# Alexandre-nk-Perdereau/video-fingerprint

Measured on NVIDIA B200. Metric: fingerprint videos/s (64 frames@64^2), higher is better.
Workload: dtype bf16

## Files before the change

### video_fingerprint_b200/csrc/stem_common.cuh

```cuda
#pragma once
#include "conv1_kernel.cuh"
#include "epilogues.cuh"

namespace vfp {

constexpr int kStemThreads = 768;
constexpr int kStemEpiWarp0 = 4, kStemEpiWarps = 8;
constexpr int kStemABuf = 9 * 16 * 128;
constexpr int kStemUnitBytes = 2 * kStemABuf;
constexpr int kStemWBlocks = 5;
constexpr int kStemRawSlotBytes = 8192;
constexpr int kStemTilePitch = 72;
constexpr int kStemTileBytes = 29184;
static_assert((67 * kStemTilePitch + 8) * 6 <= kStemTileBytes, "HWC tile");

template <int N> __device__ __forceinline__ void setmaxnreg_inc() { asm volatile("setmaxnreg.inc.sync.aligned.u32 %0;" ::"n"(N)); }
template <int N> __device__ __forceinline__ void setmaxnreg_dec() { asm volatile("setmaxnreg.dec.sync.aligned.u32 %0;" ::"n"(N)); }

__device__ __forceinline__ uint32_t relu_pack_bf16x2(float lo, float hi) {
  uint32_t d;
  asm("cvt.rn.relu.bf16x2.f32 %0, %1, %2;" : "=r"(d) : "f"(hi), "f"(lo));
  return d;
}
__device__ __forceinline__ void bulk_copy_g2s(void* dst, const void* src, uint32_t bytes, uint64_t* bar) {
  asm volatile("cp.async.bulk.shared::cluster.global.mbarrier::complete_tx::bytes [%0], [%1], %2, [%3];" ::"r"(smem_u32(dst)),
               "l"(reinterpret_cast<uint64_t>(src)), "r"(bytes), "r"(smem_u32(bar))
               : "memory");
}
__device__ __forceinline__ void bulk_prefetch_l2(const void* src, uint32_t bytes) {
  asm volatile("cp.async.bulk.prefetch.L2.global [%0], %1;" ::"l"(reinterpret_cast<uint64_t>(src)), "r"(bytes) : "memory");
}
__device__ __forceinline__ uint32_t u8x2_to_bf16x2(uint32_t lo, uint32_t hi) {
  return pack_bf16x2((float)lo * (1.0f / 255.0f), (float)hi * (1.0f / 255.0f));
}

__device__ __forceinline__ void stem_transpose_frame(const uint8_t* const (&pl)[3], uint8_t* tile, int frame_dtype, int ltid,
                                                     int n_threads) {
  if (frame_dtype == kFrameBF16) {
    for (int i = ltid; i < 512; i += n_threads) {
      const int h = i >> 3, w0 = (i & 7) * 8;
      const uint4 a = *reinterpret_cast<const uint4*>(pl[0] + (h * 64 + w0) * 2);
      const uint4 b = *reinterpret_cast<const uint4*>(pl[1] + (h * 64 + w0) * 2);
      const uint4 c = *reinterpret_cast<const uint4*>(pl[2] + (h * 64 + w0) * 2);
      uint4* dst = reinterpret_cast<uint4*>(tile + (h + 2) * (kStemTilePitch * 6) + (w0 + 8) * 6);
      uint4 o0, o1, o2;
      o0.x = __byte_perm(a.x, b.x, 0x5410); o0.y = __byte_perm(c.x, a.x, 0x7610); o0.z = __byte_perm(b.x, c.x, 0x7632);
      o0.w = __byte_perm(a.y, b.y, 0x5410); o1.x = __byte_perm(c.y, a.y, 0x7610); o1.y = __byte_perm(b.y, c.y, 0x7632);
      o1.z = __byte_perm(a.z, b.z, 0x5410); o1.w = __byte_perm(c.z, a.z, 0x7610); o2.x = __byte_perm(b.z, c.z, 0x7632);
      o2.y = __byte_perm(a.w, b.w, 0x5410); o2.z = __byte_perm(c.w, a.w, 0x7610); o2.w = __byte_perm(b.w, c.w, 0x7632);
      dst[0] = o0; dst[1] = o1; dst[2] = o2;
    }
  } else if (frame_dtype == kFrameU8) {
    for (int i = ltid; i < 512; i += n_threads) {
      const int h = i >> 3, w0 = (i & 7) * 8;
      const uint2 a = *reinterpret_cast<const uint2*>(pl[0] + h * 64 + w0);
      const uint2 b = *reinterpret_cast<const uint2*>(pl[1] + h * 64 + w0);
      const uint2 c = *reinterpret_cast<const uint2*>(pl[2] + h * 64 + w0);
      uint4* dst = reinterpret_cast<uint4*>(tile + (h + 2) * (kStemTilePitch * 6) + (w0 + 8) * 6);
      uint32_t o[12];
#pragma unroll
      for (int half = 0; half < 2; ++half) {
        const uint32_t av = half ? a.y : a.x, bv = half ? b.y : b.x, cv = half ? c.y : c.x;
#pragma unroll
        for (int pp = 0; pp < 2; ++pp) {
          const uint32_t a0 = (av >> (16 * pp)) & 0xFF, a1 = (av >> (16 * pp + 8)) & 0xFF;
          const uint32_t b0 = (bv >> (16 * pp)) & 0xFF, b1 = (bv >> (16 * pp + 8)) & 0xFF;
          const uint32_t c0 = (cv >> (16 * pp)) & 0xFF, c1 = (cv >> (16 * pp + 8)) & 0xFF;
          o[half * 6 + pp * 3 + 0] = u8x2_to_bf16x2(a0, b0);
          o[half * 6 + pp * 3 + 1] = u8x2_to_bf16x2(c0, a1);
          o[half * 6 + pp * 3 + 2] = u8x2_to_bf16x2(b1, c1);
        }
      }
      dst[0] = make_uint4(o[0], o[1], o[2], o[3]);
      dst[1] = make_uint4(o[4], o[5], o[6], o[7]);
      dst[2] = make_uint4(o[8], o[9], o[10], o[11]);
    }
  } else {
    for (int i = ltid; i < 768; i += n_threads) {
      const int byte0 = i * 16;
      const int chunk = byte0 >> 12;
      const uint4 q = *reinterpret_cast<const uint4*>((chunk == 0 ? pl[0] : chunk == 1 ? pl[1] : pl[2]) + (byte0 & 4095));
      const int h = byte0 / 192, off = byte0 - h * 192;
      uint4* dst = reinterpret_cast<uint4*>(tile + (h + 2) * (kStemTilePitch * 6) + 48 + 2 * off);
      const uint32_t w[4] = {q.x, q.y, q.z, q.w};
      uint32_t o[8];
#pragma unroll
      for (int j = 0; j < 4; ++j) {
        o[2 * j] = u8x2_to_bf16x2(w[j] & 0xFF, (w[j] >> 8) & 0xFF);
        o[2 * j + 1] = u8x2_to_bf16x2((w[j] >> 16) & 0xFF, w[j] >> 24);
      }
      dst[0] = make_uint4(o[0], o[1], o[2], o[3]);
      dst[1] = make_uint4(o[4], o[5], o[6], o[7]);
    }
  }
}

}
```

### video_fingerprint_b200/csrc/stem_ts_kernel.cuh

```cuda
#pragma once
#include "stem_common.cuh"

namespace vfp {

constexpr int kTsGenWarp0 = 12, kTsGenWarps = 4;
constexpr int kTsEpiWarp0 = 16, kTsEpiWarps = 4;
constexpr int kTsRawSlots = 3;
constexpr int kTsXposeWarp1 = 20, kTsXposeWarps = 5;
constexpr int kTsABufs = 2;
constexpr int kTsColAcc = 0, kTsColA = 256, kTsColD = 384;
#ifndef VFP_STEM_HALFB
#define VFP_STEM_HALFB 0
#endif
#ifndef VFP_STEM_KNOCKOUT
#define VFP_STEM_KNOCKOUT 0
#endif
constexpr int kTsKnock = VFP_STEM_KNOCKOUT;

struct StemTsSmem {
  static constexpr int kC1 = 0;
  static constexpr int kW2 = kC1 + 2 * kStemUnitBytes;
  static constexpr int kW1 = kW2 + kStemWBlocks * 8192;
  static constexpr int kStage = kW1 + 2 * 8192;
  static constexpr int kRaw = kStage + kStemEpiWarps * 2048;
  static constexpr int kTile = kRaw + kTsRawSlots * kStemRawSlotBytes;
  static constexpr int kBars = kTile + 2 * kStemTileBytes;
  static constexpr int kBias = kBars + 512;
  static constexpr int kTotal = kBias + 256 + 1024;
};
static_assert(StemTsSmem::kTotal <= 232448, "stem TS kernel shared memory");
static_assert(StemTsSmem::kW2 % 1024 == 0 && StemTsSmem::kW1 % 1024 == 0 && StemTsSmem::kStage % 1024 == 0 && StemTsSmem::kRaw % 1024 == 0,
              "alignment");

struct StemTsParams {
  alignas(64) CUtensorMap tmap_w2;
  alignas(64) CUtensorMap tmap_w1;
  alignas(64) CUtensorMap tmap_out;
  const unsigned long long* frame_addr;
  int frame_dtype;
  long long n_frames;
  const float* c2_bias;
};

constexpr uint32_t kDescHiSw128 = (uint32_t)(((8ull * 128) >> 4) | (1ull << 14) | (2ull << 29));
__device__ __forceinline__ uint32_t desc_lo_sw128(uint32_t smem_addr) { return ((smem_addr & 0x3FFFFu) >> 4) | (1u << 16); }

template <bool ACC>
__device__ __forceinline__ void umma_ss_lo(uint32_t tmem_d, uint32_t adesc_lo, uint32_t bdesc_lo, uint32_t idesc) {
  asm volatile(
      "{\n\t"
      ".reg .pred p;\n\t"
      ".reg .b64 da, db;\n\t"
      "setp.ne.b32 p, %5, 0;\n\t"
      "mov.b64 da, {%1, %4};\n\t"
      "mov.b64 db, {%2, %4};\n\t"
      "tcgen05.mma.cta_group::1.kind::f16 [%0], da, db, %3, p;\n\t"
      "}\n" ::"r"(tmem_d),
      "r"(adesc_lo), "r"(bdesc_lo), "r"(idesc), "r"(kDescHiSw128), "r"(ACC ? 1u : 0u)
      : "memory");
}
template <bool ACC>
__device__ __forceinline__ void umma_ts_lo(uint32_t tmem_d, uint32_t tmem_a, uint32_t bdesc_lo, uint32_t idesc) {
  asm volatile(
      "{\n\t"
      ".reg .pred p;\n\t"
      ".reg .b64 db;\n\t"
      "setp.ne.b32 p, %5, 0;\n\t"
      "mov.b64 db, {%2, %4};\n\t"
      "tcgen05.mma.cta_group::1.kind::f16 [%0], [%1], db, %3, p;\n\t"
      "}\n" ::"r"(tmem_d),
      "r"(tmem_a), "r"(bdesc_lo), "r"(idesc), "r"(kDescHiSw128), "r"(ACC ? 1u : 0u)
      : "memory");
}
__device__ __forceinline__ void tmem_st_32x32(uint32_t taddr, const uint32_t* v) {
  asm volatile(
      "tcgen05.st.sync.aligned.32x32b.x32.b32 [%0], "
      "{%1, %2, %3, %4, %5, %6, %7, %8, %9, %10, %11, %12, %13, %14, %15, %16, "
      "%17, %18, %19, %20, %21, %22, %23, %24, %25, %26, %27, %28, %29, %30, %31, %32};" ::"r"(taddr),
      "r"(v[0]), "r"(v[1]), "r"(v[2]), "r"(v[3]), "r"(v[4]), "r"(v[5]), "r"(v[6]), "r"(v[7]), "r"(v[8]), "r"(v[9]), "r"(v[10]),
      "r"(v[11]), "r"(v[12]), "r"(v[13]), "r"(v[14]), "r"(v[15]), "r"(v[16]), "r"(v[17]), "r"(v[18]), "r"(v[19]), "r"(v[20]),
      "r"(v[21]), "r"(v[22]), "r"(v[23]), "r"(v[24]), "r"(v[25]), "r"(v[26]), "r"(v[27]), "r"(v[28]), "r"(v[29]), "r"(v[30]),
      "r"(v[31])
      : "memory");
}
__device__ __forceinline__ void tmem_st_wait() { asm volatile("tcgen05.wait::st.sync.aligned;" ::: "memory"); }

__global__ void __launch_bounds__(kStemThreads, 1) stem_ts_kernel(const __grid_constant__ StemTsParams p) {
  extern __shared__ uint8_t smem_raw[];
  uint8_t* smem = smem_raw + ((1024u - (smem_u32(smem_raw) & 1023u)) & 1023u);
  uint8_t* c1buf = smem + StemTsSmem::kC1;
  uint8_t* w2buf = smem + StemTsSmem::kW2;
  uint8_t* w1buf = smem + StemTsSmem::kW1;
  uint8_t* stagebuf = smem + StemTsSmem::kStage;
  uint8_t* rawbuf = smem + StemTsSmem::kRaw;
  uint8_t* tilebuf = smem + StemTsSmem::kTile;
  uint64_t* bars = reinterpret_cast<uint64_t*>(smem + StemTsSmem::kBars);
  uint64_t* w_full = bars;
  uint64_t* c1_full = bars + 1;
  uint64_t* c1_empty = bars + 3;
  uint64_t* acc_full = bars + 28;
  uint64_t* acc_empty = bars + 30;
  uint64_t* tile_full = bars + 7;
  uint64_t* tile_empty = bars + 9;
  uint64_t* a_full = bars + 11;
  uint64_t* a_empty = bars + 14;
  uint64_t* d_full = bars + 17;
  uint64_t* d_empty = bars + 19;
  uint64_t* raw_full = bars + 32;
  uint64_t* raw_empty = bars + 37;
  uint32_t* tmem_slot = reinterpret_cast<uint32_t*>(bars + 42);
  float* c2_bias_s = reinterpret_cast<float*>(smem + StemTsSmem::kBias);

  const int tid = threadIdx.x;
  const int warp = tid >> 5, lane = tid & 31;
  pdl_launch_dependents();
  const int n_local = (p.n_frames > blockIdx.x) ? (int)((p.n_frames - blockIdx.x + gridDim.x - 1) / gridDim.x) : 0;
  const int n_tiles = 4 * n_local, n_units = 2 * n_local;

  for (int i = tid; i < (2 * kStemUnitBytes) / 16; i += kStemThreads) reinterpret_cast<uint4*>(c1buf)[i] = make_uint4(0, 0, 0, 0);
  for (int i = tid; i < (2 * kStemTileBytes) / 16; i += kStemThreads) reinterpret_cast<uint4*>(tilebuf)[i] = make_uint4(0, 0, 0, 0);
  if (tid < 64) c2_bias_s[tid] = __ldg(p.c2_bias + tid);
  if (warp == 0 && lane == 0) {
    tma_prefetch_desc(&p.tmap_w2);
    tma_prefetch_desc(&p.tmap_w1);
    tma_prefetch_desc(&p.tmap_out);
    mbar_init(w_full, 1);
    mbar_init(&c1_full[0], 2 * kTsEpiWarps);
    mbar_init(&c1_full[1], 2 * kTsEpiWarps + 1);
    for (int i = 0; i < 2; ++i) {
      mbar_init(&c1_empty[i], 1);
      mbar_init(&acc_full[i], 1);
      mbar_init(&acc_empty[i], kStemEpiWarps);
      mbar_init(&tile_full[i], kTsXposeWarps);
      mbar_init(&tile_empty[i], kTsGenWarps);
      mbar_init(&d_full[i], 1);
      mbar_init(&d_empty[i], kTsEpiWarps);
    }
    for (int i = 0; i < kTsABufs; ++i) {
      mbar_init(&a_full[i], kTsGenWarps);
      mbar_init(&a_empty[i], 1);
    }
    for (int i = 0; i < kTsRawSlots; ++i) {
      mbar_init(&raw_full[i], 1);
      mbar_init(&raw_empty[i], kTsXposeWarps);
    }
    fence_mbar_init();
  }
  if (warp == 1) {
    tmem_alloc(tmem_slot, 512);
    tmem_relinquish();
  }
  fence_proxy_async_smem();
  tc_fence_before();
  __syncthreads();
  tc_fence_after();
  const uint32_t tmem_base = *tmem_slot;
  const uint32_t plane_bytes = p.frame_dtype == kFrameBF16 ? 8192u : 4096u;
  pdl_wait();

  auto transposer_role = [&](int ltid) {
    int slot0 = 0;
    uint32_t n0 = 0;
    for (int li = 0; li < n_local; ++li) {
      const int t = li & 1;
      uint8_t* tile = tilebuf + t * kStemTileBytes;
      mbar_wait_lazy(&tile_empty[t], (uint32_t)(((li >> 1) & 1) ^ 1));
      const uint8_t* pl[3];
#pragma unroll
      for (int c = 0; c < 3; ++c) {
        const uint32_t n = n0 + c;
        const int s = (slot0 + c) % kTsRawSlots;
        mbar_wait_lazy(&raw_full[s], (n / kTsRawSlots) & 1u);
        pl[c] = rawbuf + s * kStemRawSlotBytes;
      }
      if (!(kTsKnock & 2)) stem_transpose_frame(pl, tile, p.frame_dtype, ltid, kTsXposeWarps * 32);
      __syncwarp();
      if (lane == 0) {
#pragma unroll
        for (int c = 0; c < 3; ++c) mbar_arrive(&raw_empty[(slot0 + c) % kTsRawSlots]);
        mbar_arrive(&tile_full[t]);
      }
      slot0 = (slot0 + 3) % kTsRawSlots;
      n0 += 3;
    }
  };

  if (warp < kStemEpiWarp0) {
    setmaxnreg_dec<56>();
    if (warp == 0) {
      if (lane == 0) {
        mbar_arrive_expect_tx(w_full, (kStemWBlocks + 2) * 8192);
        for (int kb = 0; kb < kStemWBlocks; ++kb) tma_load_2d(&p.tmap_w2, w_full, w2buf + kb * 8192, kb * 64, 0);
        for (int kb = 0; kb < 2; ++kb) tma_load_2d(&p.tmap_w1, w_full, w1buf + kb * 8192, kb * 64, 0);
        const unsigned long long* addr = p.frame_addr + blockIdx.x;
        int slot = 0;
        uint32_t ph = 0;
        for (int li = 0; li < n_local; ++li) {
          const uint8_t* src = reinterpret_cast<const uint8_t*>(__ldg(addr + (size_t)li * gridDim.x));
          if (li + 2 < n_local && !(kTsKnock & 4))
            bulk_prefetch_l2(reinterpret_cast<const uint8_t*>(__ldg(addr + (size_t)(li + 2) * gridDim.x)), 3 * plane_bytes);
          for (int c = 0; c < 3; ++c) {
            mbar_wait_lazy(&raw_empty[slot], ph ^ 1);
            if (kTsKnock & 4) {
              mbar_arrive(&raw_full[slot]);
            } else {
              mbar_arrive_expect_tx(&raw_full[slot], plane_bytes);
              bulk_copy_g2s(rawbuf + slot * kStemRawSlotBytes, src + c * plane_bytes, plane_bytes, &raw_full[slot]);
            }
            if (++slot == kTsRawSlots) { slot = 0; ph ^= 1; }
          }
        }
      }
    } else if (warp == 1) {
      constexpr uint32_t idesc64 = umma_idesc_bf16(128, VFP_STEM_HALFB ? 32 : 64);
      mbar_wait_relaxed(w_full, 0);
      const uint32_t w1_lo = desc_lo_sw128(smem_u32(w1buf));
      int ab = 0;
      uint32_t aph = 0;
      for (int g = 0; g < n_tiles; ++g) {
        const int b = g & 1;
        const uint32_t ph = (uint32_t)((g >> 1) & 1);
        mbar_wait_relaxed(&a_full[ab], aph);
        mbar_wait_relaxed(&d_empty[b], ph ^ 1);
        tc_fence_after();
        if (lane == 0) {
          const uint32_t a_col = tmem_base + kTsColA + ab * 64, d_col = tmem_base + kTsColD + b * 64;
          if (!(kTsKnock & 16)) {
            umma_ts_lo<false>(d_col, a_col, w1_lo, idesc64);
#pragma unroll
            for (int s = 1; s < 8; ++s) umma_ts_lo<true>(d_col, a_col + 8 * s, w1_lo + (s >> 2) * 512 + 2 * (s & 3), idesc64);
          }
          umma_commit(&a_empty[ab]);
          umma_commit(&d_full[b]);
        }
        __syncwarp();
        if (++ab == kTsABufs) { ab = 0; aph ^= 1; }
      }
    } else if (warp == 3) {
      constexpr uint32_t idesc64 = umma_idesc_bf16(128, VFP_STEM_HALFB ? 32 : 64);
      constexpr uint32_t idesc128 = umma_idesc_bf16(128, VFP_STEM_HALFB ? 64 : 128);
      mbar_wait_relaxed(w_full, 0);
      const uint32_t w2_lo = desc_lo_sw128(smem_u32(w2buf));
      const uint32_t c1_lo = desc_lo_sw128(smem_u32(c1buf));
      for (int u = 0; u < n_units; ++u) {
        const int b = u & 1;
        const uint32_t ph = (uint32_t)((u >> 1) & 1);
        mbar_wait_relaxed(&acc_empty[b], ph ^ 1);
        mbar_wait_relaxed(&c1_full[b], ph);
        tc_fence_after();
        if (lane == 0) {
          const uint32_t d_acc = tmem_base + kTsColAcc + b * 128;
          const uint32_t al0 = c1_lo + b * (kStemUnitBytes >> 4), al1 = al0 + (kStemABuf >> 4);
          if (!(kTsKnock & 8)) {
            umma_ss_lo<false>(d_acc, al1 + 128, w2_lo + 512, idesc128);
            umma_ss_lo<true>(d_acc, al0 + 128, w2_lo, idesc64);
#pragma unroll
            for (int k = 1; k < 4; ++k) {
              umma_ss_lo<true>(d_acc, al0 + 128 + 2 * k, w2_lo + 2 * k, idesc64);
              umma_ss_lo<true>(d_acc, al1 + 128 + 2 * k, w2_lo + 512 + 2 * k, idesc128);
            }
#pragma unroll
            for (int k = 0; k < 2; ++k) {
              umma_ss_lo<true>(d_acc, al0 + 2 * (2 + k), w2_lo + 3 * 512 + 2 * (2 + k), idesc64);
              umma_ss_lo<true>(d_acc, al1 + 2 * k, w2_lo + 3 * 512 + 2 * k, idesc128);
            }
          }
          umma_commit(&c1_empty[b]);
          umma_commit(&acc_full[b]);
        }
        __syncwarp();
      }
    } else {
      transposer_role(lane);
    }
  } else if (warp < kTsGenWarp0) {
    setmaxnreg_dec<56>();
    const int quarter = warp & 3;
    const int col_half = (warp - kStemEpiWarp0) >> 2;
    const float keep = (lane & 15) == 0 ? 0.0f : 1.0f;
    const float2 keep2 = make_float2(keep, keep);
    const uint32_t taddr = tmem_base + (static_cast<uint32_t>(quarter * 32) << 16) + kTsColAcc + col_half * 32;
    uint8_t* dst = stagebuf + (warp - kStemEpiWarp0) * 2048;
    uint8_t* r0 = dst + lane * 64;
    const int sw = (lane >> 1) & 3;
    int out_row = (int)blockIdx.x * 256 + quarter * 32;
    for (int u = 0; u < n_units; ++u) {
      const int b = u & 1;
      mbar_wait_relaxed(&acc_full[b], (uint32_t)((u >> 1) & 1));
      tc_fence_after();
      if (lane == 0) tma_store_wait_read<0>();
      __syncwarp();
      if (kTsKnock & 128) {
        tc_fence_before();
        __syncwarp();
        if (lane == 0) mbar_arrive(&acc_empty[b]);
        continue;
      }
      uint32_t va[2][8], vb[2][8];
      tmem_ld_32x8(taddr + b * 128, va[0]);
      tmem_ld_32x8(taddr + b * 128 + 64, vb[0]);
#pragma unroll
      for (int c = 0; c < 4; ++c) {
        uint32_t(&v0)[8] = va[c & 1];
        uint32_t(&v2)[8] = vb[c & 1];
        tmem_ld_wait();
        if (c < 3) {
          tmem_ld_32x8(taddr + b * 128 + 8 * (c + 1), va[(c + 1) & 1]);
          tmem_ld_32x8(taddr + b * 128 + 64 + 8 * (c + 1), vb[(c + 1) & 1]);
        } else {
          tc_fence_before();
          __syncwarp();
          if (lane == 0) mbar_arrive(&acc_empty[b]);
        }
        uint32_t q[4];
#pragma unroll
        for (int i = 0; i < 8; i += 4) {
          const float4 bb = *reinterpret_cast<const float4*>(c2_bias_s + col_half * 32 + 8 * c + i);
          const float s0 = __shfl_up_sync(0xffffffffu, __uint_as_float(v2[i]), 1), s1 = __shfl_up_sync(0xffffffffu, __uint_as_float(v2[i + 1]), 1);
          const float s2 = __shfl_up_sync(0xffffffffu, __uint_as_float(v2[i + 2]), 1), s3 = __shfl_up_sync(0xffffffffu, __uint_as_float(v2[i + 3]), 1);
          const float2 y01 = ffma2(make_float2(s0, s1), keep2, fadd2(make_float2(__uint_as_float(v0[i]), __uint_as_float(v0[i + 1])), make_float2(bb.x, bb.y)));
          const float2 y23 = ffma2(make_float2(s2, s3), keep2, fadd2(make_float2(__uint_as_float(v0[i + 2]), __uint_as_float(v0[i + 3])), make_float2(bb.z, bb.w)));
          q[i / 2] = relu_pack_bf16x2(y01.x, y01.y);
          q[i / 2 + 1] = relu_pack_bf16x2(y23.x, y23.y);
        }
        *reinterpret_cast<uint4*>(r0 + ((c ^ sw) << 4)) = make_uint4(q[0], q[1], q[2], q[3]);
      }
      fence_proxy_async_smem();
      __syncwarp();
      if (lane == 0 && !(kTsKnock & 1)) {
        tma_store_2d(&p.tmap_out, dst, col_half * 32, out_row + (u & 1) * 128);
        tma_store_commit();
      }
      if (u & 1) out_row += (int)gridDim.x * 256;
    }
    if (lane == 0) tma_store_wait_read<0>();
  } else if (warp < kTsEpiWarp0) {
    setmaxnreg_inc<112>();
    const int q = warp & 3;
    const int cx = lane & 15, sh = lane >> 4;
    const uint32_t lane_base = tmem_base + (static_cast<uint32_t>(q * 32) << 16) + kTsColA;
    const uint8_t* lane_src = tilebuf + ((4 * q + 2 * sh) * 108 + 6 * cx + 8) * 4;
    int ab = 0;
    uint32_t aph = 0;
    for (int li = 0; li < n_local; ++li) {
      mbar_wait_relaxed(&tile_full[li & 1], (uint32_t)((li >> 1) & 1));
#pragma unroll 1
      for (int t = 0; t < 4; ++t) {
        const uint2* src = reinterpret_cast<const uint2*>(lane_src + (li & 1) * kStemTileBytes + t * (16 * 108 * 4));
        uint32_t v[64];
#pragma unroll
        for (int kh = 0; kh < 5; ++kh)
#pragma unroll
          for (int j = 0; j < 6; ++j) {
            const uint2 w = (kTsKnock & 64) ? make_uint2(0u, 0u) : src[kh * 54 + j];
            v[kh * 12 + 2 * j] = w.x;
            v[kh * 12 + 2 * j + 1] = w.y;
          }
        v[60] = 0x3F803F80u;
        v[61] = 0u; v[62] = 0u; v[63] = 0u;
        if (t == 3) {
          __syncwarp();
          if (lane == 0) mbar_arrive(&tile_empty[li & 1]);
        }
        mbar_wait_relaxed(&a_empty[ab], aph ^ 1);
        tc_fence_after();
        if (!(kTsKnock & 512)) {
          tmem_st_32x32(lane_base + ab * 64, v);
          tmem_st_32x32(lane_base + ab * 64 + 32, v + 32);
          tmem_st_wait();
        }
        tc_fence_before();
        __syncwarp();
        if (lane == 0) mbar_arrive(&a_full[ab]);
        if (++ab == kTsABufs) { ab = 0; aph ^= 1; }
      }
    }
  } else if (warp < kTsEpiWarp0 + kTsEpiWarps) {
    setmaxnreg_inc<96>();
    const int q = warp & 3;
    const int cx = lane & 15, sh = lane >> 4;
    const uint32_t lane_base = tmem_base + (static_cast<uint32_t>(q * 32) << 16) + kTsColD;
    const uint32_t phase = (uint32_t)(cx & 7);
    uint32_t chunk_off[2][4];
#pragma unroll
    for (int sw = 0; sw < 2; ++sw)
#pragma unroll
      for (int j = 0; j < 4; ++j) chunk_off[sw][j] = (((uint32_t)((sh ^ sw) * 4 + j)) ^ phase) << 4;
    for (int g = 0; g < n_tiles; ++g) {
      const int li = g >> 2;
      const int b = g & 1;
      const int hf = (g >> 1) & 1;
      const int cyu = 4 * (g & 1) + q;
      mbar_wait_relaxed(&d_full[b], (uint32_t)((g >> 1) & 1));
      tc_fence_after();
      uint32_t packed[2][16];
#pragma unroll
      for (int sw = 0; sw < 2; ++sw) {
        if (kTsKnock & 256) break;
        uint32_t d[32];
        tmem_ld_32x32(lane_base + b * 64 + sw * 32, d);
        tmem_ld_wait();
#pragma unroll
        for (int j = 0; j < 16; ++j) packed[sw][j] = relu_pack_bf16x2(__uint_as_float(d[2 * j]), __uint_as_float(d[2 * j + 1]));
      }
      tc_fence_before();
      __syncwarp();
      if (lane == 0) mbar_arrive(&d_empty[b]);
      mbar_wait_relaxed(&c1_empty[hf], (uint32_t)((li & 1) ^ 1));
      uint8_t* row = c1buf + hf * kStemUnitBytes + ((cyu + 1) * 16 + cx) * 128;
      if (!(kTsKnock & 32)) {
#pragma unroll
        for (int sw = 0; sw < 2; ++sw)
#pragma unroll
          for (int j = 0; j < 4; ++j)
            *reinterpret_cast<uint4*>(row + sw * kStemABuf + chunk_off[sw][j]) =
                make_uint4(packed[sw][4 * j], packed[sw][4 * j + 1], packed[sw][4 * j + 2], packed[sw][4 * j + 3]);
      }
      const bool halo = hf == 0 && cyu == 7;
      if (halo) {
        mbar_wait_relaxed(&c1_empty[1], (uint32_t)((li & 1) ^ 1));
        uint8_t* hrow = c1buf + kStemUnitBytes + cx * 128;
#pragma unroll
        for (int sw = 0; sw < 2; ++sw)
#pragma unroll
          for (int j = 0; j < 4; ++j)
            *reinterpret_cast<uint4*>(hrow + sw * kStemABuf + chunk_off[sw][j]) =
                make_uint4(packed[sw][4 * j], packed[sw][4 * j + 1], packed[sw][4 * j + 2], packed[sw][4 * j + 3]);
      }
      fence_proxy_async_smem();
      __syncwarp();
      if (lane == 0) {
        mbar_arrive(&c1_full[hf]);
        if (halo) mbar_arrive(&c1_full[1]);
      }
    }
  } else {
    setmaxnreg_dec<56>();
    transposer_role((1 + warp - kTsXposeWarp1) * 32 + lane);
  }

  __syncwarp();
  tc_fence_before();
  __syncthreads();
  if (warp == 1) {
    tc_fence_after();
    tmem_dealloc(tmem_base, 512);
  }
}

}
```

### video_fingerprint_b200/csrc/vfp_b200.cu

```cuda
#include "../../include/vfp_b200.h"

#include <math.h>
#include <string.h>

#include <map>
#include <mutex>
#include <string>
#include <vector>

#include "conv1_kernel.cuh"
#include "attention_tc_kernel.cuh"
#include "conv3_ts_kernel.cuh"
#include "ffn_kernel.cuh"
#include "gemm_launch.cuh"
#include "join_kernels.cuh"
#include "metrics_kernels.cuh"
#include "model3d_kernels.cuh"
#include "preprocess_kernels.cuh"
#include "stem_ts_kernel.cuh"
#include "token_kernels.cuh"
#include "topk_kernels.cuh"

using namespace vfp;

// ... 374 lines not shown
  for (void* p : w->allocs) cudaFree(p);
  delete w;
}

int vfp_weights_embedding_dim(const vfp_weights* w) { return w ? w->embedding_dim : 0; }

int vfp_weights_create(const vfp_tensor_desc* tensors, int n_tensors, vfp_weights** out) {
  if (!tensors || !out) return fail("vfp_weights_create: null argument");
  if (vfp_device_sm_count() <= 0) return fail("vfp_weights_create: no CUDA device (there is no CPU fallback)");
  if (!tensor_map_encoder()) return fail("vfp_weights_create: cuTensorMapEncodeTiled not available from the driver");
  TensorTable t;
  for (int i = 0; i < n_tensors; ++i) t.by_name[tensors[i].name] = &tensors[i];
  std::string err;
  vfp_weights* w = new vfp_weights();
  auto bail = [&](const std::string& m) {
    vfp_weights_destroy(w);
    return fail("vfp_weights_create: " + (m.empty() ? g_last_error : m));
  };
  const std::string enc = "spatial_encoder.encoder.";

  {
    const float* cw = t.get(enc + "0.weight", 32 * 3 * 25, &err);
    const float* cb = cw ? t.get(enc + "0.bias", 32, &err) : nullptr;
    BnFold bn;
    if (!cb || !load_bn(t, enc + "1", 32, &bn, &err)) return bail(err);
    auto wk = [&](int co, int kh, int k) -> float {
      if (k >= 15) return 0.0f;
      const int kw = k / 3, c = k % 3;
      return cw[((co * 3 + c) * 5 + kh) * 5 + kw] * bn.scale[co];
    };
    std::vector<uint32_t> pack(5 * 4 * 32 * 2);
    for (int kh = 0; kh < 5; ++kh)
      for (int nt = 0; nt < 4; ++nt)
        for (int lane = 0; lane < 32; ++lane) {
          const int g = lane >> 2, tig = lane & 3, co = nt * 8 + g;
          for (int r = 0; r < 2; ++r) {
            const int k0 = 2 * tig + 8 * r;
            const __nv_bfloat16 lo = __float2bfloat16(wk(co, kh, k0)), hi = __float2bfloat16(wk(co, kh, k0 + 1));
            uint16_t l16, h16;
            memcpy(&l16, &lo, 2);
            memcpy(&h16, &hi, 2);
            pack[((kh * 4 + nt) * 32 + lane) * 2 + r] = (uint32_t)l16 | ((uint32_t)h16 << 16);
          }
        }
    std::vector<float> bias(32);
    for (int co = 0; co < 32; ++co) bias[co] = cb[co] * bn.scale[co] + bn.shift[co];
    if (upload(w, pack, &w->c1_wpack) || upload(w, bias, &w->c1_bias)) return bail("");
    std::vector<float> wts((size_t)64 * 128, 0.0f);
    for (int sw = 0; sw < 2; ++sw)
      for (int co = 0; co < 32; ++co)
        for (int kh = 0; kh < 5; ++kh)
          for (int kw = 0; kw < 5; ++kw)
            for (int ci = 0; ci < 3; ++ci)
              wts[(size_t)(sw * 32 + co) * 128 + kh * 24 + 2 + 3 * (2 * sw + kw) + ci] = cw[((co * 3 + ci) * 5 + kh) * 5 + kw] * bn.scale[co];
    for (int sw = 0; sw < 2; ++sw)
      for (int co = 0; co < 32; ++co) {
        const float hi = __bfloat162float(__float2bfloat16(bias[co]));
        wts[(size_t)(sw * 32 + co) * 128 + 120] = hi;
        wts[(size_t)(sw * 32 + co) * 128 + 121] = bias[co] - hi;
      }
    if (upload(w, to_bf16(wts), &w->c1ts_w)) return bail("");
  }
  {
    const float* cw = t.get(enc + "3.weight", 64 * 32 * 9, &err);
    const float* cb = cw ? t.get(enc + "3.bias", 64, &err) : nullptr;
    BnFold bn;
    if (!cb || !load_bn(t, enc + "4", 64, &bn, &err)) return bail(err);
    std::vector<float> wf((size_t)64 * 384, 0.0f), bf(64);
    for (int co = 0; co < 64; ++co) {
      for (int kb = 0; kb < 6; ++kb)
        for (int j = 0; j < 2; ++j) {
          const int block = 2 * kConv2KBlocks[kb].c_half + j, sh = block >> 1, sw = block & 1;
          const int kh = conv2_tap_index(kConv2KBlocks[kb].dh, sh), kw = conv2_tap_index(kConv2KBlocks[kb].dw, sw);
          if (kh < 0 || kw < 0) continue;
          for (int c = 0; c < 32; ++c)
            wf[(size_t)co * 384 + kb * 64 + j * 32 + c] = cw[((co * 32 + c) * 3 + kh) * 3 + kw] * bn.scale[co];
        }
      bf[co] = cb[co] * bn.scale[co] + bn.shift[co];
    }
    if (upload(w, to_bf16(wf), &w->c2_w) || upload(w, bf, &w->c2_b)) return bail("");
    const int fused_tap[5][2][2] = {{{1, 1}, {2, 1}}, {{2, 2}, {1, 2}}, {{2, 0}, {1, 0}}, {{0, 2}, {0, 1}}, {{0, 0}, {-1, -1}}};
    std::vector<float> wfu((size_t)64 * 320, 0.0f);
    for (int co = 0; co < 64; ++co)
      for (int kb = 0; kb < 5; ++kb)
        for (int half = 0; half < 2; ++half) {
          const int kh = fused_tap[kb][half][0], kw = fused_tap[kb][half][1];
          if (kh < 0) continue;
          for (int c = 0; c < 32; ++c)
            wfu[(size_t)co * 320 + kb * 64 + half * 32 + c] = cw[((co * 32 + c) * 3 + kh) * 3 + kw] * bn.scale[co];
        }
    if (upload(w, to_bf16(wfu), &w->c2f_w)) return bail("");
  }
  if (prep_conv3x3(w, t, 6, 64, 128, &w->c3_w, &w->c3_b, &err)) return bail(err);
  if (prep_conv3x3(w, t, 9, 128, 256, &w->c4_w, &w->c4_b, &err)) return bail(err);

  {
    const int64_t s_numel = t.numel(enc + "14.bias");
    if (s_numel <= 0) return bail("missing checkpoint tensor: " + enc + "14.bias");
    const int S = (int)s_numel;
    const float* ws = t.get(enc + "14.weight", (int64_t)S * 256, &err);
    const float* bs = ws ? t.get(enc + "14.bias", S, &err) : nullptr;
    const float* wt = bs ? t.get("temporal_projection.weight", (int64_t)kDim * S, &err) : nullptr;
    const float* bt = wt ? t.get("temporal_projection.bias", kDim, &err) : nullptr;
    if (!bt) return bail(err.empty() ? "temporal_dim must be 256" : err);
    std::vector<float> wf((size_t)kDim * 256), bf(kDim);
    for (int o = 0; o < kDim; ++o) {
      for (int i = 0; i < 256; ++i) {
// ... 81 lines not shown
    for (int o = 0; o < D; ++o)
      for (int k = 0; k < kDim; ++k) w3t[(size_t)k * D + o] = w3[(size_t)o * kDim + k];
    if (prep_dense_bf16(w, wp, (size_t)kDim * kDim, &w->wpool) || prep_f32(w, bp, kDim, &w->bpool) ||
        upload(w, w0t, &w->w0t) || prep_f32(w, b0, kDim, &w->b0) || upload(w, w3t, &w->w3t) ||
        prep_f32(w, b3, (size_t)D, &w->b3))
      return bail("");
    if (D <= 256 && D % 32 == 0) {
      if (prep_dense_bf16(w, w0, (size_t)kDim * 3 * kDim, &w->w0_bf) || prep_dense_bf16(w, w3, (size_t)D * kDim, &w->w3_bf))
        return bail("");
      if (make_tmap_rows_bf16(&w->tm_head0, w->w0_bf, kDim, 3 * kDim, 3 * kDim, 256, 64) ||
          make_tmap_rows_bf16(&w->tm_head3, w->w3_bf, (uint64_t)D, kDim, kDim, 256, 64))
        return bail("tensor map encode failed (head)");
      w->head_on_tensor_cores = true;
    }
  }
  if (make_tmap_rows_bf16(&w->tm_c2, w->c2_w, 64, 384, 384, 64, 64) ||
      make_tmap_rows_bf16(&w->tm_c2f, w->c2f_w, 64, 320, 320, 64, 64) ||
      make_tmap_rows_bf16(&w->tm_c1ts, w->c1ts_w, 64, 128, 128, 64, 64) ||
      make_tmap_rows_bf16(&w->tm_c3, w->c3_w, 128, 576, 576, 128, 64) ||
      make_tmap_rows_bf16(&w->tm_c4, w->c4_w, 256, 1152, 1152, 256, 64) ||
      make_tmap_rows_bf16(&w->tm_c3h, w->c3_w, 128, 576, 576, 64, 64) ||
      make_tmap_rows_bf16(&w->tm_c4h, w->c4_w, 256, 1152, 1152, 128, 64) ||
      make_tmap_rows_bf16(&w->tm_tok, w->wtok, kDim, 256, 256, 256, 64) ||
      make_tmap_rows_bf16(&w->tm_pool, w->wpool, kDim, kDim, kDim, 256, 64))
    return bail("tensor map encode failed (weights)");
  VFP_CUDA(cudaDeviceSynchronize());
  *out = w;
  return 0;
}

size_t vfp_forward_workspace_bytes(int64_t frames_per_pass, int64_t clips_per_pass) {
  if (frames_per_pass <= 0) return 0;
  if (clips_per_pass <= 0 || clips_per_pass > frames_per_pass) clips_per_pass = frames_per_pass;
  return forward_ws_total(frames_per_pass, clips_per_pass);
}

}

namespace {

int encode_frames_pass(const vfp_weights* w, const unsigned long long* frame_addr, int frame_dtype, bool fused_ok, int64_t F,
                       __nv_bfloat16* feat_out, uint8_t* conv_ws, cudaStream_t st) {
  const ConvWs L = conv_ws_layout(F);
  __nv_bfloat16* c1a = reinterpret_cast<__nv_bfloat16*>(conv_ws + L.c1);
  __nv_bfloat16* c2a = reinterpret_cast<__nv_bfloat16*>(conv_ws + L.c2);
  __nv_bfloat16* c3a = reinterpret_cast<__nv_bfloat16*>(conv_ws + L.c3);
  CUtensorMap ta;
  const bool fused = g_fused_stem && frame_dtype != VFP_FRAME_F32 && fused_ok;
  if (fused) {
    StemTsParams sp{};
    sp.tmap_w2 = w->tm_c2f;
    sp.tmap_w1 = w->tm_c1ts;
    if (make_tmap_out(&sp.tmap_out, c2a, (uint64_t)F * 256, 64, true)) return fail("tensor map encode failed (stem out)");
    sp.frame_addr = frame_addr; sp.frame_dtype = frame_dtype; sp.n_frames = F;
    sp.c2_bias = w->c2_b;
    VFP_CUDA(ensure_dynamic_smem(reinterpret_cast<const void*>(stem_ts_kernel), StemTsSmem::kTotal));
    g_prof.launches += 1;
    const int grid = (int)std::min<int64_t>(F, persistent_grid());
    VFP_CUDA(launch_kernel(stem_ts_kernel, dim3(grid), dim3(kStemThreads), StemTsSmem::kTotal, st, sp));
    g_prof.mark(kStStemFused, st);
  }
  for (int64_t s0 = 0; s0 < F && !fused; s0 += g_stem_pass_frames) {
    const int64_t n = std::min<int64_t>(g_stem_pass_frames, F - s0);
    g_prof.launches += 2;
    {
      const long long grid = std::min<long long>(n, (long long)device_sm_count() * 10);
      conv1_stem_kernel<<<(unsigned)grid, kC1Threads, 0, st>>>(frame_addr + s0, frame_dtype, n, w->c1_wpack,
                                                              w->c1_bias, c1a);
      g_prof.mark(kStConv1, st);
    }
    {
      if (make_tmap_nhwc_bf16(&ta, c1a, n, 16, 16, 128, 64, 16, 8, 1, 1)) return fail("tensor map encode failed (conv2)");
      GemmShape s{};
      s.m_tiles = (int)(2 * n); s.n_tiles = 1; s.k_blocks = 6; s.group_m = 16; s.a_conv = 1;
      s.tiles_per_frame = 2; s.frames_per_tile = 1; s.tile_out_rows = 8; s.h_mul = 1; s.n_segments = 1;
      for (int kb = 0; kb < 6; ++kb) {
        s.tap_c_blk[kb] = (signed char)kConv2KBlocks[kb].c_half;
        s.tap_w[kb] = (signed char)kConv2KBlocks[kb].dw;
        s.tap_h[kb] = (signed char)kConv2KBlocks[kb].dh;
      }
      EpiBiasActTma<true>::Params ep{};
      if (make_tmap_out(&ep.tmap_out, c2a + (size_t)s0 * 256 * 64, (uint64_t)n * 256, 64, true)) return fail("tensor map encode failed (conv2 out)");
      ep.bias = w->c2_b; ep.N = 64; ep.act = 1;
      VFP_CUDA((launch_gemm<64, 64, 3, EpiBiasActTma<true>, 3>(ta, w->tm_c2, s, ep, st)));
      g_prof.mark(kStConv2, st);
    }
  }
  g_prof.launches += 2;
  {
    if (g_conv3_ts) {
      Conv3Params cp{};
      if (make_tmap_nhwc_bf16(&cp.tmap_in, c2a, F, 16, 16, 64, 64, 8, 8, kC3Frames, 2) || make_tmap_out(&cp.tmap_out, c3a, (uint64_t)F * 64, 128, true))
        return fail("tensor map encode failed (conv3)");
      cp.w = w->c3_w; cp.bias = w->c3_b; cp.n_tiles = (int)((F + kC3Frames - 1) / kC3Frames);
      VFP_CUDA(ensure_dynamic_smem(reinterpret_cast<const void*>(conv3_ts_kernel<7>), Conv3Smem<7>::kTotal));
      VFP_CUDA(launch_kernel(conv3_ts_kernel<7>, dim3(std::min(cp.n_tiles, persistent_grid())), dim3(kC3Threads), Conv3Smem<7>::kTotal, st, cp));
      g_prof.mark(kStConv3, st);
    } else {
    if (make_tmap_nhwc_bf16(&ta, c2a, F, 16, 16, 64, 64, 8, 8, 2, 2)) return fail("tensor map encode failed (conv3)");
    GemmShape s{};
    s.m_tiles = (int)((F + 1) / 2); s.n_tiles = 1; s.k_blocks = 9; s.group_m = 16; s.a_conv = 1;
    s.tiles_per_frame = 1; s.frames_per_tile = 2; s.tile_out_rows = 8;
    conv_taps_strided(&s, 1);
    EpiConvTransposedTma::Params ep{};
    if (make_tmap_out(&ep.tmap_out, c3a, (uint64_t)F * 64, 128, true)) return fail("tensor map encode failed (conv3 out)");
    ep.bias = w->c3_b; ep.c_out = 128; ep.pixels_per_tile = 256;
    if (g_conv_mcast & 1) VFP_CUDA((launch_gemm<128, 64, 4, EpiConvTransposedTma, 2, true, 2>(ta, w->tm_c3h, s, ep, st)));
    else VFP_CUDA((launch_gemm<128, 64, 4, EpiConvTransposedTma, 2, true>(ta, w->tm_c3, s, ep, st)));
    g_prof.mark(kStConv3, st);
    }
  }
  {
// ... 845 lines not shown
```

Before: 305,700.

## Fuse frame transpose into A-generator warps reading raw planar frames

Drops the dedicated transposer warps and the padded HWC tile stage. The A-operand generator warps now assemble im2col rows straight from the raw planar slots, with bounds masking, and the conv1 weight K ordering is rebuilt to match the new per-channel layout. The kernel is templated on frame layout so the dtype branches compile away, and each raw slot now holds a whole frame. This removes one shared-memory round trip and its barrier handshakes and frees threads and smem, but the generator warps take on more scattered loads and per-lane masking work.

```diff
diff --git a/video_fingerprint_b200/csrc/stem_common.cuh b/video_fingerprint_b200/csrc/stem_common.cuh
--- a/video_fingerprint_b200/csrc/stem_common.cuh
+++ b/video_fingerprint_b200/csrc/stem_common.cuh
@@ -4,15 +4,12 @@
 
 namespace vfp {
 
-constexpr int kStemThreads = 768;
+constexpr int kStemThreads = 640;
 constexpr int kStemEpiWarp0 = 4, kStemEpiWarps = 8;
 constexpr int kStemABuf = 9 * 16 * 128;
 constexpr int kStemUnitBytes = 2 * kStemABuf;
 constexpr int kStemWBlocks = 5;
-constexpr int kStemRawSlotBytes = 8192;
-constexpr int kStemTilePitch = 72;
-constexpr int kStemTileBytes = 29184;
-static_assert((67 * kStemTilePitch + 8) * 6 <= kStemTileBytes, "HWC tile");
+constexpr int kStemRawSlotBytes = 3 * 8192;
 
 template <int N> __device__ __forceinline__ void setmaxnreg_inc() { asm volatile("setmaxnreg.inc.sync.aligned.u32 %0;" ::"n"(N)); }
 template <int N> __device__ __forceinline__ void setmaxnreg_dec() { asm volatile("setmaxnreg.dec.sync.aligned.u32 %0;" ::"n"(N)); }
@@ -34,65 +31,4 @@
   return pack_bf16x2((float)lo * (1.0f / 255.0f), (float)hi * (1.0f / 255.0f));
 }
 
-__device__ __forceinline__ void stem_transpose_frame(const uint8_t* const (&pl)[3], uint8_t* tile, int frame_dtype, int ltid,
-                                                     int n_threads) {
-  if (frame_dtype == kFrameBF16) {
-    for (int i = ltid; i < 512; i += n_threads) {
-      const int h = i >> 3, w0 = (i & 7) * 8;
-      const uint4 a = *reinterpret_cast<const uint4*>(pl[0] + (h * 64 + w0) * 2);
-      const uint4 b = *reinterpret_cast<const uint4*>(pl[1] + (h * 64 + w0) * 2);
-      const uint4 c = *reinterpret_cast<const uint4*>(pl[2] + (h * 64 + w0) * 2);
-      uint4* dst = reinterpret_cast<uint4*>(tile + (h + 2) * (kStemTilePitch * 6) + (w0 + 8) * 6);
-      uint4 o0, o1, o2;
-      o0.x = __byte_perm(a.x, b.x, 0x5410); o0.y = __byte_perm(c.x, a.x, 0x7610); o0.z = __byte_perm(b.x, c.x, 0x7632);
-      o0.w = __byte_perm(a.y, b.y, 0x5410); o1.x = __byte_perm(c.y, a.y, 0x7610); o1.y = __byte_perm(b.y, c.y, 0x7632);
-      o1.z = __byte_perm(a.z, b.z, 0x5410); o1.w = __byte_perm(c.z, a.z, 0x7610); o2.x = __byte_perm(b.z, c.z, 0x7632);
-      o2.y = __byte_perm(a.w, b.w, 0x5410); o2.z = __byte_perm(c.w, a.w, 0x7610); o2.w = __byte_perm(b.w, c.w, 0x7632);
-      dst[0] = o0; dst[1] = o1; dst[2] = o2;
-    }
-  } else if (frame_dtype == kFrameU8) {
-    for (int i = ltid; i < 512; i += n_threads) {
-      const int h = i >> 3, w0 = (i & 7) * 8;
-      const uint2 a = *reinterpret_cast<const uint2*>(pl[0] + h * 64 + w0);
-      const uint2 b = *reinterpret_cast<const uint2*>(pl[1] + h * 64 + w0);
-      const uint2 c = *reinterpret_cast<const uint2*>(pl[2] + h * 64 + w0);
-      uint4* dst = reinterpret_cast<uint4*>(tile + (h + 2) * (kStemTilePitch * 6) + (w0 + 8) * 6);
-      uint32_t o[12];
-#pragma unroll
-      for (int half = 0; half < 2; ++half) {
-        const uint32_t av = half ? a.y : a.x, bv = half ? b.y : b.x, cv = half ? c.y : c.x;
-#pragma unroll
-        for (int pp = 0; pp < 2; ++pp) {
-          const uint32_t a0 = (av >> (16 * pp)) & 0xFF, a1 = (av >> (16 * pp + 8)) & 0xFF;
-          const uint32_t b0 = (bv >> (16 * pp)) & 0xFF, b1 = (bv >> (16 * pp + 8)) & 0xFF;
-          const uint32_t c0 = (cv >> (16 * pp)) & 0xFF, c1 = (cv >> (16 * pp + 8)) & 0xFF;
-          o[half * 6 + pp * 3 + 0] = u8x2_to_bf16x2(a0, b0);
-          o[half * 6 + pp * 3 + 1] = u8x2_to_bf16x2(c0, a1);
-          o[half * 6 + pp * 3 + 2] = u8x2_to_bf16x2(b1, c1);
-        }
-      }
-      dst[0] = make_uint4(o[0], o[1], o[2], o[3]);
-      dst[1] = make_uint4(o[4], o[5], o[6], o[7]);
-      dst[2] = make_uint4(o[8], o[9], o[10], o[11]);
-    }
-  } else {
-    for (int i = ltid; i < 768; i += n_threads) {
-      const int byte0 = i * 16;
-      const int chunk = byte0 >> 12;
-      const uint4 q = *reinterpret_cast<const uint4*>((chunk == 0 ? pl[0] : chunk == 1 ? pl[1] : pl[2]) + (byte0 & 4095));
-      const int h = byte0 / 192, off = byte0 - h * 192;
-      uint4* dst = reinterpret_cast<uint4*>(tile + (h + 2) * (kStemTilePitch * 6) + 48 + 2 * off);
-      const uint32_t w[4] = {q.x, q.y, q.z, q.w};
-      uint32_t o[8];
-#pragma unroll
-      for (int j = 0; j < 4; ++j) {
-        o[2 * j] = u8x2_to_bf16x2(w[j] & 0xFF, (w[j] >> 8) & 0xFF);
-        o[2 * j + 1] = u8x2_to_bf16x2((w[j] >> 16) & 0xFF, w[j] >> 24);
-      }
-      dst[0] = make_uint4(o[0], o[1], o[2], o[3]);
-      dst[1] = make_uint4(o[4], o[5], o[6], o[7]);
-    }
-  }
 }
-
-}
diff --git a/video_fingerprint_b200/csrc/stem_ts_kernel.cuh b/video_fingerprint_b200/csrc/stem_ts_kernel.cuh
--- a/video_fingerprint_b200/csrc/stem_ts_kernel.cuh
+++ b/video_fingerprint_b200/csrc/stem_ts_kernel.cuh
@@ -5,8 +5,7 @@
 
 constexpr int kTsGenWarp0 = 12, kTsGenWarps = 4;
 constexpr int kTsEpiWarp0 = 16, kTsEpiWarps = 4;
-constexpr int kTsRawSlots = 3;
-constexpr int kTsXposeWarp1 = 20, kTsXposeWarps = 5;
+constexpr int kTsRawSlots = 2;
 constexpr int kTsABufs = 2;
 constexpr int kTsColAcc = 0, kTsColA = 256, kTsColD = 384;
 #ifndef VFP_STEM_HALFB
@@ -23,8 +22,7 @@
   static constexpr int kW1 = kW2 + kStemWBlocks * 8192;
   static constexpr int kStage = kW1 + 2 * 8192;
   static constexpr int kRaw = kStage + kStemEpiWarps * 2048;
-  static constexpr int kTile = kRaw + kTsRawSlots * kStemRawSlotBytes;
-  static constexpr int kBars = kTile + 2 * kStemTileBytes;
+  static constexpr int kBars = kRaw + kTsRawSlots * kStemRawSlotBytes;
   static constexpr int kBias = kBars + 512;
   static constexpr int kTotal = kBias + 256 + 1024;
 };
@@ -37,7 +35,6 @@
   alignas(64) CUtensorMap tmap_w1;
   alignas(64) CUtensorMap tmap_out;
   const unsigned long long* frame_addr;
-  int frame_dtype;
   long long n_frames;
   const float* c2_bias;
 };
@@ -85,6 +82,65 @@
 }
 __device__ __forceinline__ void tmem_st_wait() { asm volatile("tcgen05.wait::st.sync.aligned;" ::: "memory"); }
 
+__device__ __forceinline__ uint32_t lds32(const uint8_t* a) { return *reinterpret_cast<const uint32_t*>(a); }
+__device__ __forceinline__ uint32_t byte_of(uint32_t w, int i) { return (w >> (8 * i)) & 0xFFu; }
+
+template <int kLayout>
+__device__ __forceinline__ void stem_build_row(const uint8_t* slot, int r0, int cx, int sh, uint32_t (&v)[64]) {
+  const bool has_left = cx > 0, has_right = cx < 15;
+#pragma unroll
+  for (int kh = 0; kh < 5; ++kh) {
+    const int r = r0 + kh;
+    const int rc = min(max(r, 0), 63);
+    const uint32_t rm = (unsigned)r < 64u ? ~0u : 0u;
+    if constexpr (kLayout == kFrameBF16) {
+      const bool ok_a = sh ? has_right : has_left, ok_b = sh ? has_left : has_right;
+      const int off_a = !ok_a ? 8 * cx : sh ? 8 * cx + 8 : 8 * cx - 4;
+      const int off_b = !ok_b ? 8 * cx : sh ? 8 * cx - 4 : 8 * cx + 8;
+      const uint32_t ma = ok_a ? rm : 0u, mb = ok_b ? rm : 0u;
+#pragma unroll
+      for (int c = 0; c < 3; ++c) {
+        const uint8_t* row = slot + c * 8192 + rc * 128;
+        const uint32_t a = lds32(row + off_a) & ma;
+        const uint2 m = *reinterpret_cast<const uint2*>(row + 8 * cx);
+        const uint32_t b = lds32(row + off_b) & mb;
+        v[kh * 12 + 4 * c + 0] = sh ? b : a;
+        v[kh * 12 + 4 * c + 1] = m.x & rm;
+        v[kh * 12 + 4 * c + 2] = m.y & rm;
+        v[kh * 12 + 4 * c + 3] = sh ? a : b;
+      }
+    } else if constexpr (kLayout == kFrameU8) {
+      const uint32_t m0 = has_left ? rm : 0u, m2 = has_right ? rm : 0u;
+#pragma unroll
+      for (int c = 0; c < 3; ++c) {
+        const uint8_t* row = slot + c * 4096 + rc * 64 + 4 * cx;
+        const uint32_t w0 = lds32(has_left ? row - 4 : row) & m0, w1 = lds32(row) & rm, w2 = lds32(has_right ? row + 4 : row) & m2;
+        v[kh * 12 + 4 * c + 0] = u8x2_to_bf16x2(byte_of(w0, 2), byte_of(w0, 3));
+        v[kh * 12 + 4 * c + 1] = u8x2_to_bf16x2(byte_of(w1, 0), byte_of(w1, 1));
+        v[kh * 12 + 4 * c + 2] = u8x2_to_bf16x2(byte_of(w1, 2), byte_of(w1, 3));
+        v[kh * 12 + 4 * c + 3] = u8x2_to_bf16x2(byte_of(w2, 0), byte_of(w2, 1));
+      }
+    } else {
+      static_assert(kLayout == kFrameU8HWC, "frame layout");
+      const uint8_t* row = slot + rc * 192 + 12 * cx - 8;
+      uint32_t w[7];
+#pragma unroll
+      for (int j = 0; j < 7; ++j) {
+        const bool ok = j < 2 ? has_left : j < 5 ? true : has_right;
+        w[j] = lds32(row + (ok ? 4 * j : 8)) & (ok ? rm : 0u);
+      }
+#pragma unroll
+      for (int c = 0; c < 3; ++c)
+#pragma unroll
+        for (int j = 0; j < 4; ++j) {
+          const int o0 = 2 + 3 * (2 * j) + c, o1 = o0 + 3;
+          v[kh * 12 + 4 * c + j] = u8x2_to_bf16x2(byte_of(w[o0 >> 2], o0 & 3), byte_of(w[o1 >> 2], o1 & 3));
+        }
+    }
+  }
+}
+
+template <int kLayout>
 __global__ void __launch_bounds__(kStemThreads, 1) stem_ts_kernel(const __grid_constant__ StemTsParams p) {
   extern __shared__ uint8_t smem_raw[];
   uint8_t* smem = smem_raw + ((1024u - (smem_u32(smem_raw) & 1023u)) & 1023u);
@@ -93,15 +149,12 @@
   uint8_t* w1buf = smem + StemTsSmem::kW1;
   uint8_t* stagebuf = smem + StemTsSmem::kStage;
   uint8_t* rawbuf = smem + StemTsSmem::kRaw;
-  uint8_t* tilebuf = smem + StemTsSmem::kTile;
   uint64_t* bars = reinterpret_cast<uint64_t*>(smem + StemTsSmem::kBars);
   uint64_t* w_full = bars;
   uint64_t* c1_full = bars + 1;
   uint64_t* c1_empty = bars + 3;
   uint64_t* acc_full = bars + 28;
   uint64_t* acc_empty = bars + 30;
-  uint64_t* tile_full = bars + 7;
-  uint64_t* tile_empty = bars + 9;
   uint64_t* a_full = bars + 11;
   uint64_t* a_empty = bars + 14;
   uint64_t* d_full = bars + 17;
@@ -118,7 +171,6 @@
   const int n_tiles = 4 * n_local, n_units = 2 * n_local;
 
   for (int i = tid; i < (2 * kStemUnitBytes) / 16; i += kStemThreads) reinterpret_cast<uint4*>(c1buf)[i] = make_uint4(0, 0, 0, 0);
-  for (int i = tid; i < (2 * kStemTileBytes) / 16; i += kStemThreads) reinterpret_cast<uint4*>(tilebuf)[i] = make_uint4(0, 0, 0, 0);
   if (tid < 64) c2_bias_s[tid] = __ldg(p.c2_bias + tid);
   if (warp == 0 && lane == 0) {
     tma_prefetch_desc(&p.tmap_w2);
@@ -131,8 +183,6 @@
       mbar_init(&c1_empty[i], 1);
       mbar_init(&acc_full[i], 1);
       mbar_init(&acc_empty[i], kStemEpiWarps);
-      mbar_init(&tile_full[i], kTsXposeWarps);
-      mbar_init(&tile_empty[i], kTsGenWarps);
       mbar_init(&d_full[i], 1);
       mbar_init(&d_empty[i], kTsEpiWarps);
     }
@@ -142,7 +192,7 @@
     }
     for (int i = 0; i < kTsRawSlots; ++i) {
       mbar_init(&raw_full[i], 1);
-      mbar_init(&raw_empty[i], kTsXposeWarps);
+      mbar_init(&raw_empty[i], kTsGenWarps);
     }
     fence_mbar_init();
   }
@@ -155,35 +205,8 @@
   __syncthreads();
   tc_fence_after();
   const uint32_t tmem_base = *tmem_slot;
-  const uint32_t plane_bytes = p.frame_dtype == kFrameBF16 ? 8192u : 4096u;
+  constexpr uint32_t plane_bytes = kLayout == kFrameBF16 ? 8192u : 4096u;
   pdl_wait();
-
-  auto transposer_role = [&](int ltid) {
-    int slot0 = 0;
-    uint32_t n0 = 0;
-    for (int li = 0; li < n_local; ++li) {
-      const int t = li & 1;
-      uint8_t* tile = tilebuf + t * kStemTileBytes;
-      mbar_wait_lazy(&tile_empty[t], (uint32_t)(((li >> 1) & 1) ^ 1));
-      const uint8_t* pl[3];
-#pragma unroll
-      for (int c = 0; c < 3; ++c) {
-        const uint32_t n = n0 + c;
-        const int s = (slot0 + c) % kTsRawSlots;
-        mbar_wait_lazy(&raw_full[s], (n / kTsRawSlots) & 1u);
-        pl[c] = rawbuf + s * kStemRawSlotBytes;
-      }
-      if (!(kTsKnock & 2)) stem_transpose_frame(pl, tile, p.frame_dtype, ltid, kTsXposeWarps * 32);
-      __syncwarp();
-      if (lane == 0) {
-#pragma unroll
-        for (int c = 0; c < 3; ++c) mbar_arrive(&raw_empty[(slot0 + c) % kTsRawSlots]);
-        mbar_arrive(&tile_full[t]);
-      }
-      slot0 = (slot0 + 3) % kTsRawSlots;
-      n0 += 3;
-    }
-  };
 
   if (warp < kStemEpiWarp0) {
     setmaxnreg_dec<56>();
@@ -199,16 +222,15 @@
           const uint8_t* src = reinterpret_cast<const uint8_t*>(__ldg(addr + (size_t)li * gridDim.x));
           if (li + 2 < n_local && !(kTsKnock & 4))
             bulk_prefetch_l2(reinterpret_cast<const uint8_t*>(__ldg(addr + (size_t)(li + 2) * gridDim.x)), 3 * plane_bytes);
-          for (int c = 0; c < 3; ++c) {
-            mbar_wait_lazy(&raw_empty[slot], ph ^ 1);
-            if (kTsKnock & 4) {
-              mbar_arrive(&raw_full[slot]);
-            } else {
-              mbar_arrive_expect_tx(&raw_full[slot], plane_bytes);
-              bulk_copy_g2s(rawbuf + slot * kStemRawSlotBytes, src + c * plane_bytes, plane_bytes, &raw_full[slot]);
-            }
-            if (++slot == kTsRawSlots) { slot = 0; ph ^= 1; }
+          mbar_wait_lazy(&raw_empty[slot], ph ^ 1);
+          if (kTsKnock & 4) {
+            mbar_arrive(&raw_full[slot]);
+          } else {
+            mbar_arrive_expect_tx(&raw_full[slot], 3 * plane_bytes);
+            for (int c = 0; c < 3; ++c)
+              bulk_copy_g2s(rawbuf + slot * kStemRawSlotBytes + c * plane_bytes, src + c * plane_bytes, plane_bytes, &raw_full[slot]);
           }
+          if (++slot == kTsRawSlots) { slot = 0; ph ^= 1; }
         }
       }
     } else if (warp == 1) {
@@ -270,8 +292,6 @@
         }
         __syncwarp();
       }
-    } else {
-      transposer_role(lane);
     }
   } else if (warp < kTsGenWarp0) {
     setmaxnreg_dec<56>();
@@ -339,28 +359,24 @@
     const int q = warp & 3;
     const int cx = lane & 15, sh = lane >> 4;
     const uint32_t lane_base = tmem_base + (static_cast<uint32_t>(q * 32) << 16) + kTsColA;
-    const uint8_t* lane_src = tilebuf + ((4 * q + 2 * sh) * 108 + 6 * cx + 8) * 4;
-    int ab = 0;
-    uint32_t aph = 0;
+    int ab = 0, slot = 0;
+    uint32_t aph = 0, rph = 0;
     for (int li = 0; li < n_local; ++li) {
-      mbar_wait_relaxed(&tile_full[li & 1], (uint32_t)((li >> 1) & 1));
+      mbar_wait_relaxed(&raw_full[slot], rph);
 #pragma unroll 1
       for (int t = 0; t < 4; ++t) {
-        const uint2* src = reinterpret_cast<const uint2*>(lane_src + (li & 1) * kStemTileBytes + t * (16 * 108 * 4));
         uint32_t v[64];
-#pragma unroll
-        for (int kh = 0; kh < 5; ++kh)
-#pragma unroll
-          for (int j = 0; j < 6; ++j) {
-            const uint2 w = (kTsKnock & 64) ? make_uint2(0u, 0u) : src[kh * 54 + j];
-            v[kh * 12 + 2 * j] = w.x;
-            v[kh * 12 + 2 * j + 1] = w.y;
-          }
+        if (kTsKnock & 64) {
+#pragma unroll
+          for (int i = 0; i < 60; ++i) v[i] = 0u;
+        } else {
+          stem_build_row<kLayout>(rawbuf + slot * kStemRawSlotBytes, 16 * t + 4 * q + 2 * sh - 2, cx, sh, v);
+        }
         v[60] = 0x3F803F80u;
         v[61] = 0u; v[62] = 0u; v[63] = 0u;
         if (t == 3) {
           __syncwarp();
-          if (lane == 0) mbar_arrive(&tile_empty[li & 1]);
+          if (lane == 0) mbar_arrive(&raw_empty[slot]);
         }
         mbar_wait_relaxed(&a_empty[ab], aph ^ 1);
         tc_fence_after();
@@ -374,6 +390,7 @@
         if (lane == 0) mbar_arrive(&a_full[ab]);
         if (++ab == kTsABufs) { ab = 0; aph ^= 1; }
       }
+      if (++slot == kTsRawSlots) { slot = 0; rph ^= 1; }
     }
   } else if (warp < kTsEpiWarp0 + kTsEpiWarps) {
     setmaxnreg_inc<96>();
@@ -434,9 +451,6 @@
         if (halo) mbar_arrive(&c1_full[1]);
       }
     }
-  } else {
-    setmaxnreg_dec<56>();
-    transposer_role((1 + warp - kTsXposeWarp1) * 32 + lane);
   }
 
   __syncwarp();
diff --git a/video_fingerprint_b200/csrc/vfp_b200.cu b/video_fingerprint_b200/csrc/vfp_b200.cu
--- a/video_fingerprint_b200/csrc/vfp_b200.cu
+++ b/video_fingerprint_b200/csrc/vfp_b200.cu
@@ -450,7 +450,7 @@
         for (int kh = 0; kh < 5; ++kh)
           for (int kw = 0; kw < 5; ++kw)
             for (int ci = 0; ci < 3; ++ci)
-              wts[(size_t)(sw * 32 + co) * 128 + kh * 24 + 2 + 3 * (2 * sw + kw) + ci] = cw[((co * 3 + ci) * 5 + kh) * 5 + kw] * bn.scale[co];
+              wts[(size_t)(sw * 32 + co) * 128 + kh * 24 + 8 * ci + 2 * sw + kw] = cw[((co * 3 + ci) * 5 + kh) * 5 + kw] * bn.scale[co];
     for (int sw = 0; sw < 2; ++sw)
       for (int co = 0; co < 32; ++co) {
         const float hi = __bfloat162float(__float2bfloat16(bias[co]));
@@ -638,12 +638,15 @@
     sp.tmap_w2 = w->tm_c2f;
     sp.tmap_w1 = w->tm_c1ts;
     if (make_tmap_out(&sp.tmap_out, c2a, (uint64_t)F * 256, 64, true)) return fail("tensor map encode failed (stem out)");
-    sp.frame_addr = frame_addr; sp.frame_dtype = frame_dtype; sp.n_frames = F;
+    sp.frame_addr = frame_addr; sp.n_frames = F;
     sp.c2_bias = w->c2_b;
-    VFP_CUDA(ensure_dynamic_smem(reinterpret_cast<const void*>(stem_ts_kernel), StemTsSmem::kTotal));
+    auto* kern = frame_dtype == VFP_FRAME_BF16 ? stem_ts_kernel<kFrameBF16>
+               : frame_dtype == VFP_FRAME_U8   ? stem_ts_kernel<kFrameU8>
+                                               : stem_ts_kernel<kFrameU8HWC>;
+    VFP_CUDA(ensure_dynamic_smem(reinterpret_cast<const void*>(kern), StemTsSmem::kTotal));
     g_prof.launches += 1;
     const int grid = (int)std::min<int64_t>(F, persistent_grid());
-    VFP_CUDA(launch_kernel(stem_ts_kernel, dim3(grid), dim3(kStemThreads), StemTsSmem::kTotal, st, sp));
+    VFP_CUDA(launch_kernel(kern, dim3(grid), dim3(kStemThreads), StemTsSmem::kTotal, st, sp));
     g_prof.mark(kStStemFused, st);
   }
   for (int64_t s0 = 0; s0 < F && !fused; s0 += g_stem_pass_frames) {
```

After: 301,400, median of 6. 0.986x the previous value.
